# donydchen/matchnerf

Hardware: AMD Instinct MI355X
Metric: rendered rays/sec (3-view, 64 samples/ray) (higher is better)
Workload: dtype f32; 1 GPU

## Files before the change

matchnerf_amd/csrc/api.cpp:

```cpp
#include <string.h>
#include <stdarg.h>
#include <stdio.h>
#include <stdlib.h>

#include <mutex>

#include "common.hpp"
#include "launch_plan.hpp"

static thread_local char g_err[512] = "";

void mnerf_set_error(const char* fmt, ...) {
  va_list ap;
  va_start(ap, fmt);
  vsnprintf(g_err, sizeof(g_err), fmt, ap);
  va_end(ap);
}

extern "C" int mnerf_abi_version(void) { return MNERF_ABI_VERSION; }
extern "C" const char* mnerf_last_error(void) { return g_err; }

extern "C" int64_t mnerf_struct_size(int32_t which) {
  switch (which) {
    case 0: return (int64_t)sizeof(mnerf_view);
    case 1: return (int64_t)sizeof(mnerf_rays);
    case 2: return (int64_t)sizeof(mnerf_scene);
    case 3: return (int64_t)sizeof(mnerf_decoder);
    case 4: return (int64_t)sizeof(mnerf_encoder_layer);
    case 5: return (int64_t)sizeof(mnerf_conv);
    case 6: return (int64_t)sizeof(mnerf_decoder_train);
    case 7: return (int64_t)sizeof(mnerf_encoder_layer_train);
    case 8: return (int64_t)sizeof(mnerf_optim_row);
    case 9: return (int64_t)sizeof(mnerf_optim_group);
    case 10: return (int64_t)sizeof(mnerf_lpips_weights);
    case MNERF_STRUCT_CAMERA: return (int64_t)sizeof(mnerf_camera);
    default: return -1;
  }
}

int mnerf_rays_canonical(const mnerf_rays* rays, mnerf_rays* out, const char* who) {
  MNERF_REQUIRE(rays, MNERF_E_NULL, "%s: rays is NULL", who);
  *out = *rays;
  MNERF_REQUIRE(rays->tgt_height >= 0 && rays->tgt_width >= 0 && (rays->tgt_height == 0) == (rays->tgt_width == 0), MNERF_E_RANGE,
                "%s: target grid %dx%d (both 0 = the views' size, or both >= 1)", who, rays->tgt_height, rays->tgt_width);
  if (rays->tgt_height == 0) out->tgt_height = rays->height, out->tgt_width = rays->width;
  MNERF_REQUIRE(out->tgt_height >= 1 && out->tgt_width >= 1, MNERF_E_RANGE, "%s: target grid %dx%d", who, out->tgt_height,
                out->tgt_width);
  if (!rays->ray_idx && !rays->pose_table && rays->n_rays > 0)
    MNERF_REQUIRE(rays->ray_begin >= 0 && (long long)rays->ray_begin + rays->n_rays <= (long long)out->tgt_height * out->tgt_width,
                  MNERF_E_RANGE, "%s: pixels [%d, %d + %d) outside the %dx%d target grid", who, rays->ray_begin, rays->ray_begin,
                  rays->n_rays, out->tgt_height, out->tgt_width);
  return MNERF_OK;
}

int mnerf_free_rays_canonical(const mnerf_rays* rays, const float* ray_od, mnerf_rays* out, const char* who) {
  MNERF_REQUIRE(rays, MNERF_E_NULL, "%s: rays is NULL", who);
  MNERF_REQUIRE(!rays->ray_idx && !rays->pose_table, MNERF_E_UNSUPPORTED,
                "%s: a ray bundle excludes ray_idx / pose_table (the bundle's rows are the rays)", who);
  MNERF_REQUIRE(rays->n_rays >= 0 && rays->n_samples >= 1, MNERF_E_RANGE, "%s: n_rays=%d S=%d", who, rays->n_rays, rays->n_samples);
  MNERF_REQUIRE(rays->legacy_coord == 0 || rays->n_samples >= 2, MNERF_E_RANGE, "%s: legacy depth sampling needs S >= 2", who);
  if (rays->n_rays > 0) {
    MNERF_REQUIRE(ray_od, MNERF_E_NULL, "%s: ray_od is NULL", who);
    MNERF_REQUIRE(mnerf_aligned16(ray_od), MNERF_E_ALIGN, "%s: ray_od not 16B aligned", who);
  }
  mnerf_rays c = {};
  c.n_rays = rays->n_rays, c.n_samples = rays->n_samples;
  c.legacy_coord = rays->legacy_coord ? 1 : 0, c.depth_inverse = rays->depth_inverse ? 1 : 0;
  c.height = c.tgt_height = rays->height, c.width = c.tgt_width = rays->width;
  c.near_ = rays->near_, c.far_ = rays->far_;
  c.strat_u = rays->strat_u;
  *out = c;
  return MNERF_OK;
}

static int env_int(const char* name, int dflt) {
  const char* e = getenv(name);
  return (e && *e) ? atoi(e) : dflt;
}

static mnerf_tuning read_tuning() {
  mnerf_tuning t;
  t.decoder_grid = env_int("MNERF_DECODER_GRID", 512);
  t.decoder_stagger = env_int("MNERF_DECODER_STAGGER", 16);
  t.decoder_stagger_mode = env_int("MNERF_DECODER_STAGGER_MODE", 0);
  t.cv_variant = env_int("MNERF_CV_VARIANT", 3);
  t.cv_mm = env_int("MNERF_CV_MM", 1);
  t.cv_mm_spw = env_int("MNERF_CV_MM_SPW", 4);
  t.cv_uvpair = env_int("MNERF_CV_UVPAIR", -1);
  t.cv_pair_block = env_int("MNERF_CV_PAIR_BLOCK", -1);
  t.cv_grid = env_int("MNERF_CV_GRID", 0);
  t.wa_min4 = env_int("MNERF_WA_MIN4", 200);
  t.wa_xcd = env_int("MNERF_WA_XCD", 1);
  t.render_fused = env_int("MNERF_RENDER_FUSED", 0);
  t.decoder_pp = env_int("MNERF_DECODER_PP", 1);
  t.decoder_pp_grid = env_int("MNERF_DECODER_PP_GRID", 256);
  t.decoder_pp_max_s = env_int("MNERF_DECODER_PP_MAX_S", 256);
  return t;
}

static mnerf_tuning g_tuning = read_tuning();
static std::mutex g_tuning_lock;
mnerf_tuning mnerf_tune() {
  std::lock_guard<std::mutex> hold(g_tuning_lock);
  return g_tuning;
}

extern "C" int mnerf_debug_set_knob(const char* name, int value, int* old_value) {
  std::lock_guard<std::mutex> hold(g_tuning_lock);
  struct Knob { const char* name; int* slot; };
  const Knob knobs[] = {{"decoder_pp", &g_tuning.decoder_pp}, {"decoder_pp_grid", &g_tuning.decoder_pp_grid},
                        {"decoder_pp_max_s", &g_tuning.decoder_pp_max_s}, {"decoder_grid", &g_tuning.decoder_grid},
                        {"cv_variant", &g_tuning.cv_variant}, {"cv_mm", &g_tuning.cv_mm}, {"cv_mm_spw", &g_tuning.cv_mm_spw}, {"cv_uvpair", &g_tuning.cv_uvpair}, {"cv_pair_block", &g_tuning.cv_pair_block}, {"cv_grid", &g_tuning.cv_grid},
                        {"render_fused", &g_tuning.render_fused}, {"wa_min4", &g_tuning.wa_min4}};
  for (const Knob& k : knobs)
    if (name && strcmp(name, k.name) == 0) {
      if (old_value) *old_value = *k.slot;
      *k.slot = value;
      return MNERF_OK;
    }
  mnerf_set_error("mnerf_debug_set_knob: unknown knob '%s'", name ? name : "(null)");
  return MNERF_E_RANGE;
}

extern "C" int mnerf_debug_launch_plan(const char* what, const int64_t* args, int32_t n_args, int32_t* plan, int32_t n_plan) {
  MNERF_REQUIRE(what && args && plan, MNERF_E_NULL, "mnerf_debug_launch_plan: NULL argument");
  struct Planner { const char* name; int (*fn)(const int64_t*, int32_t, int32_t*, int32_t); };
  const Planner planners[] = {{"conv2d", mnerf_plan_conv2d}, {"conv_gemm", mnerf_plan_conv_gemm}, {"conv_wgrad", mnerf_plan_conv_wgrad},
                              {"instance_norm", mnerf_plan_instance_norm}, {"instance_norm_backward", mnerf_plan_instance_norm},
                              {"window_attention", mnerf_plan_window_attention}};
  for (const Planner& p : planners)
    if (strcmp(what, p.name) == 0) return p.fn(args, n_args, plan, n_plan);
  mnerf_set_error("mnerf_debug_launch_plan: unknown dispatcher '%s'", what);
  return MNERF_E_RANGE;
}

bool mnerf_once_per_device(std::atomic<unsigned long long>& mask) {
  int dev = 0;
  (void)hipGetDevice(&dev);
  const unsigned long long bit = 1ull << (dev & 63);
  return (mask.fetch_or(bit, std::memory_order_relaxed) & bit) == 0;
}
```

matchnerf_amd/csrc/cost_volume_mm.hip:

```cpp
#include <stdlib.h>

#include "cv_walk.hpp"

typedef _Float16 cvm_h8 __attribute__((ext_vector_type(8)));
typedef _Float16 cvm_h2 __attribute__((ext_vector_type(2)));
typedef float cvm_f2 __attribute__((ext_vector_type(2)));
typedef float cvm_f16 __attribute__((ext_vector_type(16)));
typedef unsigned cvm_u4 __attribute__((ext_vector_type(4)));

#define CVM_MAX_MAPS (MNERF_MAX_VIEWS * (MNERF_MAX_VIEWS - 1))
#define CVM_HDR_BYTES 8192
#define CVM_COL_BYTES 1024
#define CVM_TARGET_EXP 15
#define CVM_UV_MAX_VIEWS MNERF_MAX_VIEWS

struct CvmLayout {
  int nrp[2], rs[2];
  size_t map_bytes[2], off[2], total;
};

__host__ __device__ inline CvmLayout cvm_layout(const mnerf_scene& sc) {
  CvmLayout L;
  const size_t maps = (size_t)sc.n_views * (sc.n_views - 1);
  size_t o = CVM_HDR_BYTES;
  for (int s = 0; s < 2; ++s) {
    if (s < sc.n_scales) {
      L.nrp[s] = (sc.fh[s] + 1) / 2 + 1;
      L.rs[s] = sc.fw[s] + 3;
      L.map_bytes[s] = (size_t)L.nrp[s] * L.rs[s] * CVM_COL_BYTES;
    } else {
      L.nrp[s] = L.rs[s] = 0;
      L.map_bytes[s] = 0;
    }
    L.off[s] = o;
    o += L.map_bytes[s] * maps;
  }
  L.total = o;
  return L;
}

__global__ __launch_bounds__(256) void cvm_absmax_kernel(mnerf_scene sc, unsigned* __restrict__ absmax_bits) {
  const int maps = sc.n_views * (sc.n_views - 1);
  const int s = (int)blockIdx.y >= maps ? 1 : 0, m = (int)blockIdx.y - s * maps;
  const size_t n4 = (size_t)sc.fh[s] * sc.fw[s] * (FEAT_C / 4);
  const v4f* src = reinterpret_cast<const v4f*>(sc.feat[s]) + (size_t)m * n4;
  float mx = 0.0f;
  for (size_t i = (size_t)blockIdx.x * 256 + threadIdx.x; i < n4; i += (size_t)gridDim.x * 256) {
    const v4f v = src[i];
    mx = fmaxf(fmaxf(mx, fmaxf(fabsf(v.x), fabsf(v.y))), fmaxf(fabsf(v.z), fabsf(v.w)));
  }
#pragma unroll
  for (int off = 32; off > 0; off >>= 1) mx = fmaxf(mx, __shfl_xor(mx, off, 64));
  if ((threadIdx.x & 63) == 0) atomicMax(absmax_bits + s * CVM_MAX_MAPS + m, __float_as_uint(mx));
}

__device__ __forceinline__ int cvm_gain_exp(float m) {
  if (!(m > 0.0f) || !(m < 3.0e38f)) return 0;
  int e = __builtin_amdgcn_frexp_expf(m);
  e = e < -100 ? -100 : (e > 100 ? 100 : e);
  return CVM_TARGET_EXP - e;
}

__global__ __launch_bounds__(256) void cvm_split_kernel(mnerf_scene sc, char* __restrict__ opnd) {
  const CvmLayout L = cvm_layout(sc);
  const int maps = sc.n_views * (sc.n_views - 1);
  const int s = (int)blockIdx.y >= maps ? 1 : 0, m = (int)blockIdx.y - s * maps;
  const int fh = sc.fh[s], fw = sc.fw[s];
  const int cell = (int)blockIdx.x * 2 + (int)(threadIdx.x >> 7), ch = threadIdx.x & 127;
  if (cell >= L.nrp[s] * L.rs[s]) return;
  const int rp = cell / L.rs[s], x = cell - rp * L.rs[s];
  float* gain = reinterpret_cast<float*>(opnd);
  const unsigned* absmax_bits = reinterpret_cast<const unsigned*>(opnd + 2 * 2 * CVM_MAX_MAPS * 4);
  const int e = cvm_gain_exp(__uint_as_float(absmax_bits[s * CVM_MAX_MAPS + m]));
  const float g = ldexpf(1.0f, e);
  if (cell == 0 && ch == 0) {
    gain[s * CVM_MAX_MAPS + m] = g;
    gain[2 * CVM_MAX_MAPS + s * CVM_MAX_MAPS + m] = ldexpf(1.0f, -e);
  }
  const float* src = sc.feat[s] + (size_t)m * fh * fw * FEAT_C + ch;
  cvm_h2 hi, lo;
#pragma unroll
  for (int r = 0; r < 2; ++r) {
    const int y = 2 * rp + r;
    float v = 0.0f;
    if (y < fh && x < fw) v = src[((size_t)y * fw + x) * FEAT_C];
    v = v * g;
    v = fminf(fmaxf(v, -65504.0f), 65504.0f);
    const _Float16 h = (_Float16)v;
    hi[r] = h;
    lo[r] = (_Float16)(v - (float)h);
  }
  char* dst = opnd + L.off[s] + (size_t)m * L.map_bytes[s] + (size_t)cell * CVM_COL_BYTES + (size_t)ch * 4;
  *reinterpret_cast<cvm_h2*>(dst) = hi;
  *reinterpret_cast<cvm_h2*>(dst + 512) = lo;
}

__device__ __forceinline__ void cvm_swap32(float& a, float& b) {
  asm("s_nop 1\n\tv_permlane32_swap_b32_e32 %0, %1" : "+v"(a), "+v"(b));
}
__device__ __forceinline__ float cvm_fold_pair(float x, float y) {
  cvm_swap32(x, y);
  return x + y;
}

struct CvmTap {
  unsigned xy;
  unsigned c0_hi, c1_hi, c0_lo, c1_lo;
};

__device__ __forceinline__ unsigned cvm_pack_h2(float a, float b) {
  const cvm_f2 ab = {a, b};
  return __builtin_bit_cast(unsigned, __builtin_convertvector(ab, cvm_h2));
}
__device__ __forceinline__ float cvm_resid_lo(float v, unsigned hpk) {
  float r;
  asm("v_fma_mix_f32 %0, %1, 1.0, -%2 op_sel_hi:[0,0,1]" : "=v"(r) : "v"(v), "v"(hpk));
  return r;
}
__device__ __forceinline__ float cvm_resid_hi(float v, unsigned hpk) {
  float r;
  asm("v_fma_mix_f32 %0, %1, 1.0, -%2 op_sel:[0,0,1] op_sel_hi:[0,0,1]" : "=v"(r) : "v"(v), "v"(hpk));
  return r;
// ... 196 lines not shown
    cvm_f16 z;
#pragma unroll
    for (int i = 0; i < 16; ++i) z[i] = 0.0f;
    fa = cvm_mfma(l_a, wah, z);
    fb = cvm_mfma(l_b, wbh, z);
    fa = cvm_mfma(h_a, wal, fa);
    fb = cvm_mfma(h_b, wbl, fb);
    fa = cvm_mfma(h_a, wah, fa);
    fb = cvm_mfma(h_b, wbh, fb);
  };
  auto request = [&](int ct) {
    if constexpr (REQ) {
      cvm_load_ct(ha[ct], la[ct], next_a, ct);
      cvm_load_ct(hb[ct], lb[ct], next_b, ct);
    }
  };
#define CVM_PIN(q) asm volatile("" : "+v"(dot[q]), "+v"(dot[q + 1]), "+v"(na[q]), "+v"(na[q + 1]), "+v"(nb[q]), "+v"(nb[q + 1]));
  if constexpr (MORE) {
    const unsigned loff_a = cvm_lane_off(sa.rs, n, half), loff_b = cvm_lane_off(sb.rs, n, half);
#pragma unroll 1
    for (int ct = 0; ct < 4; ++ct) {
#pragma unroll
      for (int i = 0; i < 16; ++i) fa0[i] = 0.0f, fb0[i] = 0.0f;
      cvm_all_chunks(fa0, sa, tap_a, loff_a, ct, lut, half, fh, fw);
      cvm_all_chunks(fb0, sb, tap_b, loff_b, ct, lut, half, fh, fw);
      float d2[2], a2[2], b2[2];
      cvm_dots(fa0, fb0, d2, a2, b2);
      switch (ct) {
        case 0: dot[0] = d2[0], dot[1] = d2[1], na[0] = a2[0], na[1] = a2[1], nb[0] = b2[0], nb[1] = b2[1]; break;
        case 1: dot[2] = d2[0], dot[3] = d2[1], na[2] = a2[0], na[3] = a2[1], nb[2] = b2[0], nb[3] = b2[1]; break;
        case 2: dot[4] = d2[0], dot[5] = d2[1], na[4] = a2[0], na[5] = a2[1], nb[4] = b2[0], nb[5] = b2[1]; break;
        default: dot[6] = d2[0], dot[7] = d2[1], na[6] = a2[0], na[7] = a2[1], nb[6] = b2[0], nb[7] = b2[1]; break;
      }
    }
#pragma unroll
    for (int ct = 0; ct < 4; ++ct) request(ct);
  } else {
    tile(0, fa0, fb0);
    request(0);
    tile(1, fa1, fb1);
    cvm_dots(fa0, fb0, dot + 0, na + 0, nb + 0);
    CVM_PIN(0)
    request(1);
    tile(2, fa0, fb0);
    cvm_dots(fa1, fb1, dot + 2, na + 2, nb + 2);
    CVM_PIN(2)
    request(2);
    tile(3, fa1, fb1);
    cvm_dots(fa0, fb0, dot + 4, na + 4, nb + 4);
    CVM_PIN(4)
    request(3);
    cvm_dots(fa1, fb1, dot + 6, na + 6, nb + 6);
  }
#undef CVM_PIN
  cvm_cosines(cacc, dot, na, nb, ea2, eb2, G);
}


struct CvmGrid {
  int tile_y0, ntx, n_tiles, nsg, spw;
  int stage_rows;
  int pair_begin, pair_end, a0, b0;
};

__host__ __device__ inline size_t cvm_wave_lds_bytes(int n_views, int n_scales, int cond_stride, int stage_rows) {
  const size_t items = (size_t)n_views * n_scales;
  return (size_t)n_views * 32 * 8 + items * (32 * 16 + 32 * 4 + 16) + (stage_rows ? (size_t)32 * cond_stride * 4 : 0);
}

#define CVM_WAVES_PER_SIMD 2
#define CVM_WG_WAVES 4
#ifdef CVM_STATS
#define CVM_DBG_PARAM , unsigned long long* __restrict__ dbg
#define CVM_T(i)                                                  \
  {                                                               \
    const unsigned long long t_ = __builtin_amdgcn_s_memtime();   \
    st[i] += t_ - t_last;                                         \
    t_last = t_;                                                  \
  }
#else
#define CVM_DBG_PARAM
#define CVM_T(i)
#endif
__global__ __launch_bounds__(64 * CVM_WG_WAVES, CVM_WAVES_PER_SIMD) void cost_volume_mm_kernel(mnerf_scene sc, mnerf_rays R, int cond_stride,
                                                                                 float* __restrict__ cond, const char* __restrict__ opnd,
                                                                                 CvmGrid grid CVM_DBG_PARAM) {
#ifdef CVM_STATS
  unsigned long long st[8] = {0, 0, 0, 0, 0, 0, 0, 0}, t_last = __builtin_amdgcn_s_memtime();
#endif
  extern __shared__ __attribute__((aligned(16))) char cvm_smem[];
  const int lane = threadIdx.x & 63, wave = __builtin_amdgcn_readfirstlane(threadIdx.x >> 6);
  const int n = lane & 31, half = lane >> 5;
  const int S = R.n_samples, V = sc.n_views, NS = sc.n_scales;
  const int W = R.tgt_width, H = R.tgt_height;
  const int Ws = R.width, Hs = R.height;
  const int items = V * NS;
  const CvmLayout L = cvm_layout(sc);
  const float* gain = reinterpret_cast<const float*>(opnd);
  const cvm_u4* lut = reinterpret_cast<const cvm_u4*>(cvm_smem);
  cvm_lut_init(reinterpret_cast<unsigned*>(cvm_smem));
  __syncthreads();
  char* wl = cvm_smem + CVM_LUT_BYTES + (size_t)wave * cvm_wave_lds_bytes(V, NS, cond_stride, grid.stage_rows);
  float2* uv = reinterpret_cast<float2*>(wl);
  cvm_u4* tapw = reinterpret_cast<cvm_u4*>(wl + (size_t)V * 256);
  unsigned* tapxy = reinterpret_cast<unsigned*>(wl + (size_t)V * 256 + (size_t)items * 512);
  int4* boxes = reinterpret_cast<int4*>(wl + (size_t)V * 256 + (size_t)items * 640);
  float* rows = reinterpret_cast<float*>(wl + (size_t)V * 256 + (size_t)items * 656);

  const int nwg = gridDim.x;
  const int xcd = blockIdx.x & 7, lin = blockIdx.x >> 3;
  const int q8 = nwg >> 3, r8 = nwg & 7;
  const int item = (xcd < r8 ? xcd * (q8 + 1) : r8 * (q8 + 1) + (xcd - r8) * q8) + lin;
  const int tile = item / grid.nsg, sg = item - tile * grid.nsg;
  const int tyi = tile / grid.ntx, txi = tile - tyi * grid.ntx;

  const int px = txi * 8 + (n & 7), py = (grid.tile_y0 + tyi) * 4 + (n >> 3);
  const int pix = min(py, H - 1) * W + min(px, W - 1);
  const int ray_geo = pix - R.ray_begin;
  const int ray = max(0, min(ray_geo, R.n_rays - 1));
  const bool row_wr = grid.stage_rows || (px < W && py < H && ray_geo >= 0 && ray_geo < R.n_rays);
  const float wm1 = (float)(Ws - 1), hm1 = (float)(Hs - 1);
  const int G0 = sc.n_group[0], G1 = NS > 1 ? sc.n_group[1] : 0;
  const int sumG = G0 + G1;
  const int n_pairs = V * (V - 1) / 2;
  const float inv_pairs = 1.0f / (float)n_pairs;
  const bool first_block = grid.pair_begin == 0, last_block = grid.pair_end == n_pairs;

  for (int k = 0; k < grid.spw; ++k) {
    const int j = (sg * grid.spw + k) * CVM_WG_WAVES + wave;
    if (j >= S) break;
    float* out = grid.stage_rows ? rows + n * cond_stride : cond + ((size_t)ray * S + j) * cond_stride;
    float wx, wy, wz;
    {
      int rg = ray_geo;
      asm volatile("" : "+v"(rg));
      ray_point(make_ray(R, rg), sample_depth(R, ray, j), wx, wy, wz);
    }

    CVM_T(7)
    cvw_handoff();
    for (int v = half; v < V; v += 2) {
      float u, w_, z;
      project(sc.views[v], wx, wy, wz, wm1, hm1, u, w_, z);
      uv[v * 32 + n] = make_float2(u, w_);
      if (row_wr && first_block) {
        const Bilin b = bilin_setup(u, w_, Hs, Ws);
        const float4* img = reinterpret_cast<const float4*>(sc.images) + (size_t)v * Hs * Ws;
        const float4 t00 = img[b.o00], t01 = img[b.o01], t10 = img[b.o10], t11 = img[b.o11];
        const float gx = u * 2.0f - 1.0f, gy = w_ * 2.0f - 1.0f;
        const float m = (gx > -1.0f && gx < 1.0f && gy > -1.0f && gy < 1.0f) ? 1.0f : 0.0f;
        out[sumG + 3 * v + 0] = bilin4(t00.x, t01.x, t10.x, t11.x, b);
        out[sumG + 3 * v + 1] = bilin4(t00.y, t01.y, t10.y, t11.y, b);
        out[sumG + 3 * v + 2] = bilin4(t00.z, t01.z, t10.z, t11.z, b);
        out[sumG + 3 * V + v] = m;
      }
    }
    if (half == 0 && row_wr && first_block) {
      const int dc = sumG + 4 * V;
      out[dc] = 1.0f;
      for (int c = dc + 1; c < cond_stride; ++c) out[c] = 0.0f;
    }
    cvw_handoff();
    CVM_T(0)

    for (int it = 0; 2 * it < items; ++it) {
      const int i = min(2 * it + half, items - 1);
      const int v = NS == 2 ? i >> 1 : i, s = i - v * NS;
      const float2 p2 = uv[v * 32 + n];
      int x0, y0;
      const int fh_s = s == 0 ? sc.fh[0] : sc.fh[1], fw_s = s == 0 ? sc.fw[0] : sc.fw[1];
      const CvmTap t = cvm_tap(p2.x, p2.y, fh_s, fw_s, x0, y0);
      cvm_u4 wv;
      wv.x = t.c0_hi, wv.y = t.c1_hi, wv.z = t.c0_lo, wv.w = t.c1_lo;
      tapw[i * 32 + n] = wv;
      tapxy[i * 32 + n] = t.xy;
      const int y1 = min(y0 + 1, fh_s - 1), x1 = min(x0 + 1, fw_s - 1);
      int xmin = x0, ymin = y0;
#define CVM_MM_STEP(CTRL)                                                                                                    \
  {                                                                                                                          \
    xmin = min(xmin, __builtin_amdgcn_update_dpp(0x7fffffff, xmin, CTRL, 0xF, 0xF, false));  \
    ymin = min(ymin, __builtin_amdgcn_update_dpp(0x7fffffff, ymin, CTRL, 0xF, 0xF, false));                                         \
  }
      CVM_MM_STEP(0xB1)
      CVM_MM_STEP(0x4E)
      CVM_MM_STEP(0x141)
      CVM_MM_STEP(0x140)
#undef CVM_MM_STEP
      xmin = min(xmin, __builtin_amdgcn_ds_swizzle(xmin, 0x401F));
      ymin = min(ymin, __builtin_amdgcn_ds_swizzle(ymin, 0x401F));
      const int p_lo = ymin >> 1, xb_lo = xmin;
      const int cra = ((y0 >> 1) - p_lo) >> 1, crb = ((y1 >> 1) - p_lo) >> 1;
      const int cxa = (x0 - xb_lo) >> 2, cxb = (x1 - xb_lo) >> 2;
      const unsigned long long ob = __builtin_amdgcn_ballot_w64(crb > 7 || cxb > 7);
      const bool big = (half ? (unsigned)(ob >> 32) : (unsigned)ob) != 0u;
      unsigned long long mk = (1ull << ((8 * cra + cxa) & 63)) | (1ull << ((8 * cra + cxb) & 63)) | (1ull << ((8 * crb + cxa) & 63)) |
                              (1ull << ((8 * crb + cxb) & 63));
      unsigned mlo = (unsigned)mk, mhi = (unsigned)(mk >> 32);
#define CVM_OR_STEP(CTRL)                                                                             \
  {                                                                                                   \
    mlo |= (unsigned)__builtin_amdgcn_update_dpp(0, (int)mlo, CTRL, 0xF, 0xF, false);                 \
    mhi |= (unsigned)__builtin_amdgcn_update_dpp(0, (int)mhi, CTRL, 0xF, 0xF, false);                 \
  }
      CVM_OR_STEP(0xB1)
      CVM_OR_STEP(0x4E)
      CVM_OR_STEP(0x141)
      CVM_OR_STEP(0x140)
#undef CVM_OR_STEP
      mlo |= (unsigned)__builtin_amdgcn_ds_swizzle((int)mlo, 0x401F);
      mhi |= (unsigned)__builtin_amdgcn_ds_swizzle((int)mhi, 0x401F);
      if (n == 0 && 2 * it + half < items) boxes[i] = make_int4(p_lo, xb_lo, big ? 0 : (int)mlo, big ? 0 : (int)mhi);
    }
    cvw_handoff();

    CVM_T(1)
    float c0[4] = {0.f, 0.f, 0.f, 0.f}, c1[4] = {0.f, 0.f, 0.f, 0.f};
    if (!first_block && row_wr) {
#pragma unroll
      for (int i = 0; i < 4; ++i) {
        const int gi = 2 * i + half;
        if (gi < G0) c0[i] = out[gi];
        if (gi < G1) c1[i] = out[G0 + gi];
      }
    }
    auto tap_of = [&](int i) {
      CvmTap t;
      const cvm_u4 wv = tapw[i * 32 + n];
      t.xy = tapxy[i * 32 + n];
      t.c0_hi = wv.x, t.c1_hi = wv.y, t.c0_lo = wv.z, t.c1_lo = wv.w;
      return t;
    };
    auto side_of = [&](const char* map, int view, int s) {
      CvmSide o;
      o.map = map;
      o.rs = s == 0 ? L.rs[0] : L.rs[1];
      o.item = view * NS + s;
      const int4 bx = boxes[o.item];
      o.box.p_lo = __builtin_amdgcn_readfirstlane(bx.x), o.box.xb_lo = __builtin_amdgcn_readfirstlane(bx.y);
      o.box.mask = (unsigned long long)(unsigned)__builtin_amdgcn_readfirstlane(bx.z) |
                   ((unsigned long long)(unsigned)__builtin_amdgcn_readfirstlane(bx.w) << 32);
      o.box.big = o.box.mask == 0;
      o.p = o.box.p_lo, o.xb = o.box.xb_lo;
      if (!o.box.big) {
        unsigned long long m = o.box.mask;
        cvm_pop(m, o.box, o.p, o.xb);
      }
      return o;
    };
    auto first_of = [&](const CvmSide& sd) { return cvm_chunk_base(sd, sd.p, sd.xb) + cvm_lane_off(sd.rs, n, half); };
    auto has_more = [&](const CvmSide& sd) { return sd.box.big || (sd.box.mask & (sd.box.mask - 1)) != 0; };
    const char* mp0 = opnd + L.off[0] + (size_t)(2 * grid.pair_begin) * L.map_bytes[0];
    const char* mp1 = opnd + L.off[1] + (size_t)(2 * grid.pair_begin) * L.map_bytes[1];
    int pr = grid.pair_begin, a = grid.a0, b = grid.b0, s = 0;
    CvmSide sa = side_of(mp0, a, 0), sb = side_of(mp0 + L.map_bytes[0], b, 0);
    cvm_u4 ha[4], la[4], hb[4], lb[4];
    {
      const char* fa_ = first_of(sa);
      const char* fb_ = first_of(sb);
#pragma unroll
      for (int ct = 0; ct < 4; ++ct) cvm_load_ct(ha[ct], la[ct], fa_, ct), cvm_load_ct(hb[ct], lb[ct], fb_, ct);
    }
    const int n_units = (grid.pair_end - grid.pair_begin) * NS;
    auto unit = [&](auto req_tag) {
      constexpr bool REQ = decltype(req_tag)::value;
      CVM_T(2)
      const float ga = gain[s * CVM_MAX_MAPS + 2 * pr], gb = gain[s * CVM_MAX_MAPS + 2 * pr + 1];
      const float ea = 1e-8f * ga, eb = 1e-8f * gb;
      const int G = s == 0 ? G0 : G1;
      const int s_cur = s;
      const int fh_u = s == 0 ? sc.fh[0] : sc.fh[1], fw_u = s == 0 ? sc.fw[0] : sc.fw[1];
      CvmSide na_ = sa, nb_ = sb;
      if constexpr (REQ) {
        if (++s == NS) {
          s = 0, ++pr;
          mp0 += 2 * L.map_bytes[0], mp1 += 2 * L.map_bytes[1];
          if (++b == V) ++a, b = a + 1;
        }
        const char* mpn = s == 0 ? mp0 : mp1;
        na_ = side_of(mpn, a, s);
        nb_ = side_of(mpn + (s == 0 ? L.map_bytes[0] : L.map_bytes[1]), b, s);
      }
      const CvmTap tap_a = tap_of(sa.item), tap_b = tap_of(sb.item);
      float cu[4] = {0.f, 0.f, 0.f, 0.f};
      if (has_more(sa) || has_more(sb))
        cvm_unit_run<true, REQ>(cu, ha, la, hb, lb, sa, sb, tap_a, tap_b, first_of(na_), first_of(nb_), ea * ea, eb * eb, G, lut, n, half, fh_u,
                                fw_u);
      else
        cvm_unit_run<false, REQ>(cu, ha, la, hb, lb, sa, sb, tap_a, tap_b, first_of(na_), first_of(nb_), ea * ea, eb * eb, G, lut, n, half, fh_u,
                                 fw_u);
      if (s_cur == 0) {
#pragma unroll
        for (int i = 0; i < 4; ++i) c0[i] += cu[i];
      } else {
#pragma unroll
        for (int i = 0; i < 4; ++i) c1[i] += cu[i];
      }
      sa = na_, sb = nb_;
      CVM_T(5)
    };
    for (int u = 0; u + 1 < n_units; ++u) unit(std::true_type{});
    if (n_units > 0) unit(std::false_type{});
    if (row_wr) {
#pragma unroll
      for (int i = 0; i < 4; ++i) {
        const int gi = 2 * i + half;
        if (gi < G0) out[gi] = last_block ? c0[i] * inv_pairs : c0[i];
        if (gi < G1) out[G0 + gi] = last_block ? c1[i] * inv_pairs : c1[i];
      }
    }
    cvw_handoff();
    if (grid.stage_rows) {
      const int ppr = cond_stride >> 2;
      const int ppr_sh = (ppr & (ppr - 1)) == 0 ? __builtin_ctz(ppr) : -1;
      for (int c = lane; c < 32 * ppr; c += 64) {
        const int r = ppr_sh >= 0 ? c >> ppr_sh : c / ppr, part = c - r * ppr;
        const int rpx = txi * 8 + (r & 7), rpy = (grid.tile_y0 + tyi) * 4 + (r >> 3);
        const int rpix = rpy * W + rpx;
        if (rpx < W && rpy < H && rpix >= R.ray_begin && rpix < R.ray_begin + R.n_rays)
          *reinterpret_cast<v4f*>(cond + ((size_t)(rpix - R.ray_begin) * S + j) * cond_stride + 4 * part) =
              *reinterpret_cast<const v4f*>(rows + r * cond_stride + 4 * part);
      }
    }
    CVM_T(6)
  }
#ifdef CVM_STATS
  if (dbg && lane == 0) {
    for (int i = 0; i < 8; ++i) atomicAdd(dbg + i, st[i]);
    atomicAdd(dbg + 8, 1ull);
  }
#endif
}

extern "C" int64_t mnerf_cost_volume_operand_bytes(const mnerf_scene* scene) {
  if (!scene || scene->n_views < 2 || scene->n_views > MNERF_MAX_VIEWS || scene->n_scales < 1 || scene->n_scales > 2) return -1;
  return (int64_t)cvm_layout(*scene).total;
}

extern "C" int mnerf_cost_volume_operands(const mnerf_scene* scene, void* opnd, void* stream) {
  MNERF_REQUIRE(scene && opnd, MNERF_E_NULL, "mnerf_cost_volume_operands: NULL argument");
  MNERF_REQUIRE(scene->n_views >= 2 && scene->n_views <= MNERF_MAX_VIEWS, MNERF_E_RANGE, "mnerf_cost_volume_operands: n_views=%d",
                scene->n_views);
  MNERF_REQUIRE(scene->n_scales == 1 || scene->n_scales == 2, MNERF_E_RANGE, "mnerf_cost_volume_operands: n_scales=%d", scene->n_scales);
  MNERF_REQUIRE(mnerf_aligned16(opnd), MNERF_E_ALIGN, "mnerf_cost_volume_operands: buffer not 16B aligned");
  for (int s = 0; s < scene->n_scales; ++s) {
    MNERF_REQUIRE(scene->feat[s], MNERF_E_NULL, "mnerf_cost_volume_operands: feat[%d] is NULL", s);
    MNERF_REQUIRE(mnerf_aligned16(scene->feat[s]), MNERF_E_ALIGN, "mnerf_cost_volume_operands: feat[%d] not 16B aligned", s);
    MNERF_REQUIRE(scene->fh[s] >= 1 && scene->fw[s] >= 1, MNERF_E_RANGE, "mnerf_cost_volume_operands: feature map %d is %dx%d", s,
                  scene->fh[s], scene->fw[s]);
  }
  const CvmLayout L = cvm_layout(*scene);
  const int maps = scene->n_views * (scene->n_views - 1);
  hipStream_t st = (hipStream_t)stream;
  hipError_t e = hipMemsetAsync(opnd, 0, CVM_HDR_BYTES, st);
  if (e != hipSuccess) {
    mnerf_set_error("mnerf_cost_volume_operands: memset failed: %s", hipGetErrorString(e));
    return (int)e;
  }
  unsigned* absmax_bits = reinterpret_cast<unsigned*>(reinterpret_cast<char*>(opnd) + 2 * 2 * CVM_MAX_MAPS * 4);
  hipLaunchKernelGGL(cvm_absmax_kernel, dim3(32, (unsigned)(maps * scene->n_scales)), dim3(256), 0, st, *scene, absmax_bits);
  int cells = 0;
  for (int s = 0; s < scene->n_scales; ++s) cells = cells > L.nrp[s] * L.rs[s] ? cells : L.nrp[s] * L.rs[s];
  hipLaunchKernelGGL(cvm_split_kernel, dim3((unsigned)((cells + 1) / 2), (unsigned)(maps * scene->n_scales)), dim3(256), 0, st, *scene,
                     reinterpret_cast<char*>(opnd));
  return mnerf_check_launch("mnerf_cost_volume_operands");
}

bool mnerf_cost_volume_mm_applies(const mnerf_scene* scene, const mnerf_rays* rays) {
  return scene->feat_op != nullptr && rays->ray_idx == nullptr && rays->pose_table == nullptr;
}

int mnerf_cost_volume_mm_launch(const mnerf_scene* scene, const mnerf_rays* rays, int cond_stride, float* cond, void* stream) {
  MNERF_REQUIRE(mnerf_aligned16(scene->feat_op), MNERF_E_ALIGN, "mnerf_cost_volume: feat_op not 16B aligned");
  const int W = rays->tgt_width;
  const int row_first = rays->ray_begin / W, row_last = (rays->ray_begin + rays->n_rays - 1) / W;
  CvmGrid g;
  g.tile_y0 = row_first / 4;
  g.ntx = (W + 7) / 8;
  g.n_tiles = g.ntx * (row_last / 4 - g.tile_y0 + 1);
  int spw = mnerf_tune().cv_mm_spw;
  if (spw <= 0) spw = 4;
  g.spw = spw;
  g.nsg = (rays->n_samples + CVM_WG_WAVES * spw - 1) / (CVM_WG_WAVES * spw);
  const long long items = (long long)g.n_tiles * g.nsg;
  MNERF_REQUIRE(items < (1ll << 31), MNERF_E_RANGE, "mnerf_cost_volume: %lld work items", items);
  const int n_pairs = scene->n_views * (scene->n_views - 1) / 2;
  int blk = mnerf_tune().cv_pair_block > 0 ? mnerf_tune().cv_pair_block : n_pairs;
  if (scene->n_views <= 5) blk = n_pairs;
  g.stage_rows = blk >= n_pairs &&
                 (2 * (CVM_LUT_BYTES + CVM_WG_WAVES * cvm_wave_lds_bytes(scene->n_views, scene->n_scales, cond_stride, 1)) <= 160 * 1024 ||
                  2 * (CVM_LUT_BYTES + CVM_WG_WAVES * cvm_wave_lds_bytes(scene->n_views, scene->n_scales, cond_stride, 0)) > 160 * 1024);
  const size_t lds = CVM_LUT_BYTES + CVM_WG_WAVES * cvm_wave_lds_bytes(scene->n_views, scene->n_scales, cond_stride, g.stage_rows);
  MNERF_REQUIRE(lds <= 160 * 1024, MNERF_E_UNSUPPORTED, "mnerf_cost_volume: %d views need %zu B of LDS", scene->n_views, lds);
  static std::atomic<unsigned long long> attr_set{0};
  if (mnerf_once_per_device(attr_set))
    (void)hipFuncSetAttribute((const void*)cost_volume_mm_kernel, hipFuncAttributeMaxDynamicSharedMemorySize, 160 * 1024);
#ifdef CVM_STATS
  unsigned long long* dbg = nullptr;
  if (const char* e = getenv("MNERF_CVDBG_PTR")) dbg = (unsigned long long*)strtoull(e, nullptr, 0);
#endif
  int a = 0, b = 1;
  for (int p0 = 0; p0 < n_pairs; p0 += blk) {
    g.pair_begin = p0, g.pair_end = p0 + blk < n_pairs ? p0 + blk : n_pairs, g.a0 = a, g.b0 = b;
#ifdef CVM_STATS
    hipLaunchKernelGGL(cost_volume_mm_kernel, dim3((unsigned)items), dim3(64 * CVM_WG_WAVES), lds, (hipStream_t)stream, *scene, *rays,
                       cond_stride, cond, reinterpret_cast<const char*>(scene->feat_op), g, dbg);
#else
    hipLaunchKernelGGL(cost_volume_mm_kernel, dim3((unsigned)items), dim3(64 * CVM_WG_WAVES), lds, (hipStream_t)stream, *scene, *rays,
                       cond_stride, cond, reinterpret_cast<const char*>(scene->feat_op), g);
#endif
    for (int i = 0; i < blk; ++i)
      if (++b == scene->n_views) ++a, b = a + 1;
  }
  return mnerf_check_launch("mnerf_cost_volume");
}
```

matchnerf_amd/csrc/launch_plan.hpp:

```cpp
#pragma once
#include <stdint.h>

int mnerf_plan_conv2d(const int64_t* args, int32_t n_args, int32_t* plan, int32_t n_plan);
int mnerf_plan_conv_gemm(const int64_t* args, int32_t n_args, int32_t* plan, int32_t n_plan);
int mnerf_plan_conv_wgrad(const int64_t* args, int32_t n_args, int32_t* plan, int32_t n_plan);
int mnerf_plan_instance_norm(const int64_t* args, int32_t n_args, int32_t* plan, int32_t n_plan);
int mnerf_plan_window_attention(const int64_t* args, int32_t n_args, int32_t* plan, int32_t n_plan);
```

Before: 12.85 million rays/s.

## Add compile-time specialized cost-volume kernel for 3 views and 2 scales

Templates the matmul cost-volume kernel on view and scale counts and dispatches a fully static instance for the 3-view, 2-scale case. The pair and scale walk is unrolled at compile time, per-unit gain epsilons are precomputed into scalar registers, box descriptors are hoisted once, and the view projection loop is unrolled. This removes runtime index arithmetic and dynamic pair/scale bookkeeping from the inner loop. The cost is larger code and possibly more register pressure. A launch-plan query and a runtime knob are added to turn the path on or off.

```diff
diff --git a/matchnerf_amd/csrc/api.cpp b/matchnerf_amd/csrc/api.cpp
--- a/matchnerf_amd/csrc/api.cpp
+++ b/matchnerf_amd/csrc/api.cpp
@@ -104,13 +104,18 @@
   std::lock_guard<std::mutex> hold(g_tuning_lock);
   return g_tuning;
 }
+static int g_cv_mm_static = env_int("MNERF_CV_MM_STATIC", 1);
+int mnerf_cv_mm_static() {
+  std::lock_guard<std::mutex> hold(g_tuning_lock);
+  return g_cv_mm_static;
+}
 
 extern "C" int mnerf_debug_set_knob(const char* name, int value, int* old_value) {
   std::lock_guard<std::mutex> hold(g_tuning_lock);
   struct Knob { const char* name; int* slot; };
   const Knob knobs[] = {{"decoder_pp", &g_tuning.decoder_pp}, {"decoder_pp_grid", &g_tuning.decoder_pp_grid},
                         {"decoder_pp_max_s", &g_tuning.decoder_pp_max_s}, {"decoder_grid", &g_tuning.decoder_grid},
-                        {"cv_variant", &g_tuning.cv_variant}, {"cv_mm", &g_tuning.cv_mm}, {"cv_mm_spw", &g_tuning.cv_mm_spw}, {"cv_uvpair", &g_tuning.cv_uvpair}, {"cv_pair_block", &g_tuning.cv_pair_block}, {"cv_grid", &g_tuning.cv_grid},
+                        {"cv_variant", &g_tuning.cv_variant}, {"cv_mm", &g_tuning.cv_mm}, {"cv_mm_spw", &g_tuning.cv_mm_spw}, {"cv_mm_static", &g_cv_mm_static}, {"cv_uvpair", &g_tuning.cv_uvpair}, {"cv_pair_block", &g_tuning.cv_pair_block}, {"cv_grid", &g_tuning.cv_grid},
                         {"render_fused", &g_tuning.render_fused}, {"wa_min4", &g_tuning.wa_min4}};
   for (const Knob& k : knobs)
     if (name && strcmp(name, k.name) == 0) {
@@ -127,7 +132,7 @@
   struct Planner { const char* name; int (*fn)(const int64_t*, int32_t, int32_t*, int32_t); };
   const Planner planners[] = {{"conv2d", mnerf_plan_conv2d}, {"conv_gemm", mnerf_plan_conv_gemm}, {"conv_wgrad", mnerf_plan_conv_wgrad},
                               {"instance_norm", mnerf_plan_instance_norm}, {"instance_norm_backward", mnerf_plan_instance_norm},
-                              {"window_attention", mnerf_plan_window_attention}};
+                              {"window_attention", mnerf_plan_window_attention}, {"cost_volume_mm", mnerf_plan_cost_volume_mm}};
   for (const Planner& p : planners)
     if (strcmp(what, p.name) == 0) return p.fn(args, n_args, plan, n_plan);
   mnerf_set_error("mnerf_debug_launch_plan: unknown dispatcher '%s'", what);
diff --git a/matchnerf_amd/csrc/cost_volume_mm.hip b/matchnerf_amd/csrc/cost_volume_mm.hip
--- a/matchnerf_amd/csrc/cost_volume_mm.hip
+++ b/matchnerf_amd/csrc/cost_volume_mm.hip
@@ -1,6 +1,10 @@
 #include <stdlib.h>
 
+#include <type_traits>
+#include <utility>
+
 #include "cv_walk.hpp"
+#include "launch_plan.hpp"
 
 typedef _Float16 cvm_h8 __attribute__((ext_vector_type(8)));
 typedef _Float16 cvm_h2 __attribute__((ext_vector_type(2)));
@@ -19,12 +23,12 @@
   size_t map_bytes[2], off[2], total;
 };
 
-__host__ __device__ inline CvmLayout cvm_layout(const mnerf_scene& sc) {
+__host__ __device__ inline CvmLayout cvm_layout_of(const mnerf_scene& sc, int n_views, int n_scales) {
   CvmLayout L;
-  const size_t maps = (size_t)sc.n_views * (sc.n_views - 1);
+  const size_t maps = (size_t)n_views * (n_views - 1);
   size_t o = CVM_HDR_BYTES;
   for (int s = 0; s < 2; ++s) {
-    if (s < sc.n_scales) {
+    if (s < n_scales) {
       L.nrp[s] = (sc.fh[s] + 1) / 2 + 1;
       L.rs[s] = sc.fw[s] + 3;
       L.map_bytes[s] = (size_t)L.nrp[s] * L.rs[s] * CVM_COL_BYTES;
@@ -38,6 +42,7 @@
   L.total = o;
   return L;
 }
+__host__ __device__ inline CvmLayout cvm_layout(const mnerf_scene& sc) { return cvm_layout_of(sc, sc.n_views, sc.n_scales); }
 
 __global__ __launch_bounds__(256) void cvm_absmax_kernel(mnerf_scene sc, unsigned* __restrict__ absmax_bits) {
   const int maps = sc.n_views * (sc.n_views - 1);
@@ -400,20 +405,37 @@
 #define CVM_DBG_PARAM
 #define CVM_T(i)
 #endif
+struct CvmUnitDesc {
+  int a, b, s, pr;
+};
+template <int V_, int NS_>
+constexpr CvmUnitDesc cvm_unit_desc(int u) {
+  CvmUnitDesc d = {0, 1, u % NS_, u / NS_};
+  for (int i = 0; i < d.pr; ++i)
+    if (++d.b == V_) ++d.a, d.b = d.a + 1;
+  return d;
+}
+template <class F, int... I>
+__device__ __forceinline__ void cvm_each_index(F&& f, std::integer_sequence<int, I...>) {
+  (f(std::integral_constant<int, I>{}), ...);
+}
+
+template <int V_, int NS_>
 __global__ __launch_bounds__(64 * CVM_WG_WAVES, CVM_WAVES_PER_SIMD) void cost_volume_mm_kernel(mnerf_scene sc, mnerf_rays R, int cond_stride,
                                                                                  float* __restrict__ cond, const char* __restrict__ opnd,
                                                                                  CvmGrid grid CVM_DBG_PARAM) {
 #ifdef CVM_STATS
   unsigned long long st[8] = {0, 0, 0, 0, 0, 0, 0, 0}, t_last = __builtin_amdgcn_s_memtime();
 #endif
+  constexpr bool ST = V_ != 0;
   extern __shared__ __attribute__((aligned(16))) char cvm_smem[];
   const int lane = threadIdx.x & 63, wave = __builtin_amdgcn_readfirstlane(threadIdx.x >> 6);
   const int n = lane & 31, half = lane >> 5;
-  const int S = R.n_samples, V = sc.n_views, NS = sc.n_scales;
+  const int S = R.n_samples, V = ST ? V_ : sc.n_views, NS = ST ? NS_ : sc.n_scales;
   const int W = R.tgt_width, H = R.tgt_height;
   const int Ws = R.width, Hs = R.height;
   const int items = V * NS;
-  const CvmLayout L = cvm_layout(sc);
+  const CvmLayout L = cvm_layout_of(sc, V, NS);
   const float* gain = reinterpret_cast<const float*>(opnd);
   const cvm_u4* lut = reinterpret_cast<const cvm_u4*>(cvm_smem);
   cvm_lut_init(reinterpret_cast<unsigned*>(cvm_smem));
@@ -441,12 +463,30 @@
   const int G0 = sc.n_group[0], G1 = NS > 1 ? sc.n_group[1] : 0;
   const int sumG = G0 + G1;
   const int n_pairs = V * (V - 1) / 2;
-  const float inv_pairs = 1.0f / (float)n_pairs;
-  const bool first_block = grid.pair_begin == 0, last_block = grid.pair_end == n_pairs;
-
+  const float inv_pairs = 1.0f / (float)(sc.n_views * (sc.n_views - 1) / 2);
+  const bool first_block = ST || grid.pair_begin == 0, last_block = ST || grid.pair_end == n_pairs;
+  constexpr int NU = ST ? V_ * (V_ - 1) / 2 * NS_ : 1;
+  float ea2_st[NU], eb2_st[NU];
+  if constexpr (ST) {
+#pragma unroll
+    for (int u = 0; u < NU; ++u) {
+      const int slot = (u % NS_) * CVM_MAX_MAPS + 2 * (u / NS_);
+      const float ea = 1e-8f * gain[slot], eb = 1e-8f * gain[slot + 1];
+      ea2_st[u] = __builtin_bit_cast(float, __builtin_amdgcn_readfirstlane(__builtin_bit_cast(int, ea * ea)));
+      eb2_st[u] = __builtin_bit_cast(float, __builtin_amdgcn_readfirstlane(__builtin_bit_cast(int, eb * eb)));
+    }
+  }
+
+  const int n_w = n, half_w = half;
   for (int k = 0; k < grid.spw; ++k) {
     const int j = (sg * grid.spw + k) * CVM_WG_WAVES + wave;
     if (j >= S) break;
+    int n = n_w, half = half_w;
+    if constexpr (ST) {
+      int lane_k = lane;
+      asm volatile("" : "+v"(lane_k));
+      n = lane_k & 31, half = lane_k >> 5;
+    }
     float* out = grid.stage_rows ? rows + n * cond_stride : cond + ((size_t)ray * S + j) * cond_stride;
     float wx, wy, wz;
     {
@@ -457,7 +497,7 @@
 
     CVM_T(7)
     cvw_handoff();
-    for (int v = half; v < V; v += 2) {
+    auto pass1_view = [&](int v) {
       float u, w_, z;
       project(sc.views[v], wx, wy, wz, wm1, hm1, u, w_, z);
       uv[v * 32 + n] = make_float2(u, w_);
@@ -472,6 +512,17 @@
         out[sumG + 3 * v + 2] = bilin4(t00.z, t01.z, t10.z, t11.z, b);
         out[sumG + 3 * V + v] = m;
       }
+    };
+    if constexpr (ST) {
+#pragma unroll
+      for (int v0 = 0; v0 < V_; v0 += 2) {
+        if (v0 + 1 < V_)
+          pass1_view(v0 + half);
+        else if (half == 0)
+          pass1_view(v0);
+      }
+    } else {
+      for (int v = half; v < V; v += 2) pass1_view(v);
     }
     if (half == 0 && row_wr && first_block) {
       const int dc = sumG + 4 * V;
@@ -481,9 +532,7 @@
     cvw_handoff();
     CVM_T(0)
 
-    for (int it = 0; 2 * it < items; ++it) {
-      const int i = min(2 * it + half, items - 1);
-      const int v = NS == 2 ? i >> 1 : i, s = i - v * NS;
+    auto pass1b_item = [&](int i, int v, int s, bool store) {
       const float2 p2 = uv[v * 32 + n];
       int x0, y0;
       const int fh_s = s == 0 ? sc.fh[0] : sc.fh[1], fw_s = s == 0 ? sc.fw[0] : sc.fw[1];
@@ -526,7 +575,17 @@
 #undef CVM_OR_STEP
       mlo |= (unsigned)__builtin_amdgcn_ds_swizzle((int)mlo, 0x401F);
       mhi |= (unsigned)__builtin_amdgcn_ds_swizzle((int)mhi, 0x401F);
-      if (n == 0 && 2 * it + half < items) boxes[i] = make_int4(p_lo, xb_lo, big ? 0 : (int)mlo, big ? 0 : (int)mhi);
+      if (n == 0 && store) boxes[i] = make_int4(p_lo, xb_lo, big ? 0 : (int)mlo, big ? 0 : (int)mhi);
+    };
+    if constexpr (ST && NS_ == 2) {
+#pragma unroll
+      for (int it = 0; it < V_; ++it) pass1b_item(2 * it + half, it, half, true);
+    } else {
+      for (int it = 0; 2 * it < items; ++it) {
+        const int i = min(2 * it + half, items - 1);
+        const int v = NS == 2 ? i >> 1 : i, s = i - v * NS;
+        pass1b_item(i, v, s, 2 * it + half < items);
+      }
     }
     cvw_handoff();
 
@@ -547,15 +606,13 @@
       t.c0_hi = wv.x, t.c1_hi = wv.y, t.c0_lo = wv.z, t.c1_lo = wv.w;
       return t;
     };
-    auto side_of = [&](const char* map, int view, int s) {
+    auto side_of_box = [&](const char* map, int rs, int item, const int4& bx) {
       CvmSide o;
       o.map = map;
-      o.rs = s == 0 ? L.rs[0] : L.rs[1];
-      o.item = view * NS + s;
-      const int4 bx = boxes[o.item];
-      o.box.p_lo = __builtin_amdgcn_readfirstlane(bx.x), o.box.xb_lo = __builtin_amdgcn_readfirstlane(bx.y);
-      o.box.mask = (unsigned long long)(unsigned)__builtin_amdgcn_readfirstlane(bx.z) |
-                   ((unsigned long long)(unsigned)__builtin_amdgcn_readfirstlane(bx.w) << 32);
+      o.rs = rs;
+      o.item = item;
+      o.box.p_lo = bx.x, o.box.xb_lo = bx.y;
+      o.box.mask = (unsigned long long)(unsigned)bx.z | ((unsigned long long)(unsigned)bx.w << 32);
       o.box.big = o.box.mask == 0;
       o.p = o.box.p_lo, o.xb = o.box.xb_lo;
       if (!o.box.big) {
@@ -564,59 +621,137 @@
       }
       return o;
     };
+    auto side_of = [&](const char* map, int view, int s) {
+      const int4 bx = boxes[view * NS + s];
+      return side_of_box(map, s == 0 ? L.rs[0] : L.rs[1], view * NS + s,
+                         make_int4(__builtin_amdgcn_readfirstlane(bx.x), __builtin_amdgcn_readfirstlane(bx.y),
+                                   __builtin_amdgcn_readfirstlane(bx.z), __builtin_amdgcn_readfirstlane(bx.w)));
+    };
     auto first_of = [&](const CvmSide& sd) { return cvm_chunk_base(sd, sd.p, sd.xb) + cvm_lane_off(sd.rs, n, half); };
     auto has_more = [&](const CvmSide& sd) { return sd.box.big || (sd.box.mask & (sd.box.mask - 1)) != 0; };
-    const char* mp0 = opnd + L.off[0] + (size_t)(2 * grid.pair_begin) * L.map_bytes[0];
-    const char* mp1 = opnd + L.off[1] + (size_t)(2 * grid.pair_begin) * L.map_bytes[1];
-    int pr = grid.pair_begin, a = grid.a0, b = grid.b0, s = 0;
-    CvmSide sa = side_of(mp0, a, 0), sb = side_of(mp0 + L.map_bytes[0], b, 0);
     cvm_u4 ha[4], la[4], hb[4], lb[4];
-    {
-      const char* fa_ = first_of(sa);
-      const char* fb_ = first_of(sb);
-#pragma unroll
-      for (int ct = 0; ct < 4; ++ct) cvm_load_ct(ha[ct], la[ct], fa_, ct), cvm_load_ct(hb[ct], lb[ct], fb_, ct);
-    }
-    const int n_units = (grid.pair_end - grid.pair_begin) * NS;
-    auto unit = [&](auto req_tag) {
-      constexpr bool REQ = decltype(req_tag)::value;
-      CVM_T(2)
-      const float ga = gain[s * CVM_MAX_MAPS + 2 * pr], gb = gain[s * CVM_MAX_MAPS + 2 * pr + 1];
-      const float ea = 1e-8f * ga, eb = 1e-8f * gb;
-      const int G = s == 0 ? G0 : G1;
-      const int s_cur = s;
-      const int fh_u = s == 0 ? sc.fh[0] : sc.fh[1], fw_u = s == 0 ? sc.fw[0] : sc.fw[1];
-      CvmSide na_ = sa, nb_ = sb;
-      if constexpr (REQ) {
-        if (++s == NS) {
-          s = 0, ++pr;
-          mp0 += 2 * L.map_bytes[0], mp1 += 2 * L.map_bytes[1];
-          if (++b == V) ++a, b = a + 1;
+    if constexpr (ST) {
+      static_assert(NS_ == 2, "the static instance selects between a pair's two scales");
+      constexpr int NI = V_ * NS_, NP = NU / NS_;
+      int4 bxs[NI];
+#pragma unroll
+      for (int i = 0; i < NI; ++i) {
+        const int4 bx = boxes[i];
+        bxs[i].x = __builtin_amdgcn_readfirstlane(bx.x), bxs[i].y = __builtin_amdgcn_readfirstlane(bx.y);
+        bxs[i].z = __builtin_amdgcn_readfirstlane(bx.z), bxs[i].w = __builtin_amdgcn_readfirstlane(bx.w);
+      }
+      auto side_st = [&](bool first, auto ux, auto uy, auto side_tag) {
+        constexpr CvmUnitDesc X = cvm_unit_desc<V_, NS_>(decltype(ux)::value), Y = cvm_unit_desc<V_, NS_>(decltype(uy)::value);
+        constexpr int SIDE = decltype(side_tag)::value;
+        constexpr int IX = (SIDE ? X.b : X.a) * NS_ + X.s, IY = (SIDE ? Y.b : Y.a) * NS_ + Y.s;
+        const int4 bx = make_int4(first ? bxs[IX].x : bxs[IY].x, first ? bxs[IX].y : bxs[IY].y, first ? bxs[IX].z : bxs[IY].z,
+                                  first ? bxs[IX].w : bxs[IY].w);
+        const size_t mb = first ? L.map_bytes[X.s] : L.map_bytes[Y.s];
+        const char* map = opnd + (first ? L.off[X.s] : L.off[Y.s]) + (size_t)(first ? 2 * X.pr + SIDE : 2 * Y.pr + SIDE) * mb;
+        return side_of_box(map, first ? L.rs[X.s] : L.rs[Y.s], first ? IX : IY, bx);
+      };
+      using cvm_side_a = std::integral_constant<int, 0>;
+      using cvm_side_b = std::integral_constant<int, 1>;
+      {
+        using U0 = std::integral_constant<int, 0>;
+        const char* fa_ = first_of(side_st(true, U0{}, U0{}, cvm_side_a{}));
+        const char* fb_ = first_of(side_st(true, U0{}, U0{}, cvm_side_b{}));
+#pragma unroll
+        for (int ct = 0; ct < 4; ++ct) cvm_load_ct(ha[ct], la[ct], fa_, ct), cvm_load_ct(hb[ct], lb[ct], fb_, ct);
+      }
+      auto unit_st = [&](auto pr_tag, auto req_tag, int s) {
+        constexpr int PR = decltype(pr_tag)::value;
+        constexpr bool REQ = decltype(req_tag)::value;
+        using U0 = std::integral_constant<int, 2 * PR>;
+        using U1 = std::integral_constant<int, 2 * PR + 1>;
+        using U2 = std::integral_constant<int, (2 * PR + 2 < NU ? 2 * PR + 2 : NU - 1)>;
+        CVM_T(2)
+        const bool s0 = s == 0;
+        const CvmSide sa = side_st(s0, U0{}, U1{}, cvm_side_a{}), sb = side_st(s0, U0{}, U1{}, cvm_side_b{});
+        const char *next_a = nullptr, *next_b = nullptr;
+        if constexpr (REQ) {
+          next_a = first_of(side_st(s0, U1{}, U2{}, cvm_side_a{}));
+          next_b = first_of(side_st(s0, U1{}, U2{}, cvm_side_b{}));
         }
-        const char* mpn = s == 0 ? mp0 : mp1;
-        na_ = side_of(mpn, a, s);
-        nb_ = side_of(mpn + (s == 0 ? L.map_bytes[0] : L.map_bytes[1]), b, s);
-      }
-      const CvmTap tap_a = tap_of(sa.item), tap_b = tap_of(sb.item);
-      float cu[4] = {0.f, 0.f, 0.f, 0.f};
-      if (has_more(sa) || has_more(sb))
-        cvm_unit_run<true, REQ>(cu, ha, la, hb, lb, sa, sb, tap_a, tap_b, first_of(na_), first_of(nb_), ea * ea, eb * eb, G, lut, n, half, fh_u,
-                                fw_u);
-      else
-        cvm_unit_run<false, REQ>(cu, ha, la, hb, lb, sa, sb, tap_a, tap_b, first_of(na_), first_of(nb_), ea * ea, eb * eb, G, lut, n, half, fh_u,
-                                 fw_u);
-      if (s_cur == 0) {
-#pragma unroll
-        for (int i = 0; i < 4; ++i) c0[i] += cu[i];
-      } else {
-#pragma unroll
-        for (int i = 0; i < 4; ++i) c1[i] += cu[i];
-      }
-      sa = na_, sb = nb_;
-      CVM_T(5)
-    };
-    for (int u = 0; u + 1 < n_units; ++u) unit(std::true_type{});
-    if (n_units > 0) unit(std::false_type{});
+        const CvmTap tap_a = tap_of(sa.item), tap_b = tap_of(sb.item);
+        const int G = s0 ? G0 : G1;
+        const float ea2 = s0 ? ea2_st[2 * PR] : ea2_st[2 * PR + 1], eb2 = s0 ? eb2_st[2 * PR] : eb2_st[2 * PR + 1];
+        float cu[4] = {0.f, 0.f, 0.f, 0.f};
+        if (has_more(sa) || has_more(sb)) {
+          const int fh_u = s0 ? sc.fh[0] : sc.fh[1], fw_u = s0 ? sc.fw[0] : sc.fw[1];
+          cvm_unit_run<true, REQ>(cu, ha, la, hb, lb, sa, sb, tap_a, tap_b, next_a, next_b, ea2, eb2, G, lut, n, half, fh_u, fw_u);
+        } else {
+          cvm_unit_run<false, REQ>(cu, ha, la, hb, lb, sa, sb, tap_a, tap_b, next_a, next_b, ea2, eb2, G, lut, n, half, 0, 0);
+        }
+        if (s0) {
+#pragma unroll
+          for (int i = 0; i < 4; ++i) c0[i] += cu[i];
+        } else {
+#pragma unroll
+          for (int i = 0; i < 4; ++i) c1[i] += cu[i];
+        }
+        CVM_T(5)
+      };
+      cvm_each_index(
+          [&](auto pr_tag) {
+            constexpr bool LAST = decltype(pr_tag)::value == NP - 1;
+#pragma unroll 1
+            for (int s = 0; s < (LAST ? NS_ - 1 : NS_); ++s) unit_st(pr_tag, std::true_type{}, s);
+            if constexpr (LAST) unit_st(pr_tag, std::false_type{}, NS_ - 1);
+          },
+          std::make_integer_sequence<int, NP>{});
+    } else {
+      const char* mp0 = opnd + L.off[0] + (size_t)(2 * grid.pair_begin) * L.map_bytes[0];
+      const char* mp1 = opnd + L.off[1] + (size_t)(2 * grid.pair_begin) * L.map_bytes[1];
+      int pr = grid.pair_begin, a = grid.a0, b = grid.b0, s = 0;
+      CvmSide sa = side_of(mp0, a, 0), sb = side_of(mp0 + L.map_bytes[0], b, 0);
+      {
+        const char* fa_ = first_of(sa);
+        const char* fb_ = first_of(sb);
+#pragma unroll
+        for (int ct = 0; ct < 4; ++ct) cvm_load_ct(ha[ct], la[ct], fa_, ct), cvm_load_ct(hb[ct], lb[ct], fb_, ct);
+      }
+      const int n_units = (grid.pair_end - grid.pair_begin) * NS;
+      auto unit = [&](auto req_tag) {
+        constexpr bool REQ = decltype(req_tag)::value;
+        CVM_T(2)
+        const float ga = gain[s * CVM_MAX_MAPS + 2 * pr], gb = gain[s * CVM_MAX_MAPS + 2 * pr + 1];
+        const float ea = 1e-8f * ga, eb = 1e-8f * gb;
+        const int G = s == 0 ? G0 : G1;
+        const int s_cur = s;
+        const int fh_u = s == 0 ? sc.fh[0] : sc.fh[1], fw_u = s == 0 ? sc.fw[0] : sc.fw[1];
+        CvmSide na_ = sa, nb_ = sb;
+        if constexpr (REQ) {
+          if (++s == NS) {
+            s = 0, ++pr;
+            mp0 += 2 * L.map_bytes[0], mp1 += 2 * L.map_bytes[1];
+            if (++b == V) ++a, b = a + 1;
+          }
+          const char* mpn = s == 0 ? mp0 : mp1;
+          na_ = side_of(mpn, a, s);
+          nb_ = side_of(mpn + (s == 0 ? L.map_bytes[0] : L.map_bytes[1]), b, s);
+        }
+        const CvmTap tap_a = tap_of(sa.item), tap_b = tap_of(sb.item);
+        float cu[4] = {0.f, 0.f, 0.f, 0.f};
+        if (has_more(sa) || has_more(sb))
+          cvm_unit_run<true, REQ>(cu, ha, la, hb, lb, sa, sb, tap_a, tap_b, first_of(na_), first_of(nb_), ea * ea, eb * eb, G, lut, n, half, fh_u,
+                                  fw_u);
+        else
+          cvm_unit_run<false, REQ>(cu, ha, la, hb, lb, sa, sb, tap_a, tap_b, first_of(na_), first_of(nb_), ea * ea, eb * eb, G, lut, n, half, fh_u,
+                                   fw_u);
+        if (s_cur == 0) {
+#pragma unroll
+          for (int i = 0; i < 4; ++i) c0[i] += cu[i];
+        } else {
+#pragma unroll
+          for (int i = 0; i < 4; ++i) c1[i] += cu[i];
+        }
+        sa = na_, sb = nb_;
+        CVM_T(5)
+      };
+      for (int u = 0; u + 1 < n_units; ++u) unit(std::true_type{});
+      if (n_units > 0) unit(std::false_type{});
+    }
     if (row_wr) {
 #pragma unroll
       for (int i = 0; i < 4; ++i) {
@@ -684,6 +819,26 @@
 
 bool mnerf_cost_volume_mm_applies(const mnerf_scene* scene, const mnerf_rays* rays) {
   return scene->feat_op != nullptr && rays->ray_idx == nullptr && rays->pose_table == nullptr;
+}
+
+static int cvm_pair_block(int n_views) {
+  const int n_pairs = n_views * (n_views - 1) / 2;
+  int blk = mnerf_tune().cv_pair_block > 0 ? mnerf_tune().cv_pair_block : n_pairs;
+  if (n_views <= 5) blk = n_pairs;
+  return blk;
+}
+static bool cvm_takes_static(int n_views, int n_scales, int blk) {
+  return n_views == 3 && n_scales == 2 && blk >= n_views * (n_views - 1) / 2 && mnerf_cv_mm_static() != 0;
+}
+
+int mnerf_plan_cost_volume_mm(const int64_t* a, int32_t n_args, int32_t* plan, int32_t n_plan) {
+  const char* who = "mnerf_debug_launch_plan(cost_volume_mm)";
+  MNERF_REQUIRE(n_args == 2 && n_plan >= 2, MNERF_E_RANGE, "%s: takes 2 arguments and fills 2 values, got %d and %d", who, n_args, n_plan);
+  MNERF_REQUIRE(a[0] >= 2 && a[0] <= MNERF_MAX_VIEWS && (a[1] == 1 || a[1] == 2), MNERF_E_RANGE, "%s: n_views=%lld n_scales=%lld", who,
+                (long long)a[0], (long long)a[1]);
+  const int blk = cvm_pair_block((int)a[0]);
+  plan[0] = cvm_takes_static((int)a[0], (int)a[1], blk) ? 1 : 0, plan[1] = blk;
+  return MNERF_OK;
 }
 
 int mnerf_cost_volume_mm_launch(const mnerf_scene* scene, const mnerf_rays* rays, int cond_stride, float* cond, void* stream) {
@@ -701,16 +856,17 @@
   const long long items = (long long)g.n_tiles * g.nsg;
   MNERF_REQUIRE(items < (1ll << 31), MNERF_E_RANGE, "mnerf_cost_volume: %lld work items", items);
   const int n_pairs = scene->n_views * (scene->n_views - 1) / 2;
-  int blk = mnerf_tune().cv_pair_block > 0 ? mnerf_tune().cv_pair_block : n_pairs;
-  if (scene->n_views <= 5) blk = n_pairs;
+  const int blk = cvm_pair_block(scene->n_views);
   g.stage_rows = blk >= n_pairs &&
                  (2 * (CVM_LUT_BYTES + CVM_WG_WAVES * cvm_wave_lds_bytes(scene->n_views, scene->n_scales, cond_stride, 1)) <= 160 * 1024 ||
                   2 * (CVM_LUT_BYTES + CVM_WG_WAVES * cvm_wave_lds_bytes(scene->n_views, scene->n_scales, cond_stride, 0)) > 160 * 1024);
   const size_t lds = CVM_LUT_BYTES + CVM_WG_WAVES * cvm_wave_lds_bytes(scene->n_views, scene->n_scales, cond_stride, g.stage_rows);
   MNERF_REQUIRE(lds <= 160 * 1024, MNERF_E_UNSUPPORTED, "mnerf_cost_volume: %d views need %zu B of LDS", scene->n_views, lds);
-  static std::atomic<unsigned long long> attr_set{0};
-  if (mnerf_once_per_device(attr_set))
-    (void)hipFuncSetAttribute((const void*)cost_volume_mm_kernel, hipFuncAttributeMaxDynamicSharedMemorySize, 160 * 1024);
+  const bool st = cvm_takes_static(scene->n_views, scene->n_scales, blk);
+  auto* kernel = st ? cost_volume_mm_kernel<3, 2> : cost_volume_mm_kernel<0, 0>;
+  static std::atomic<unsigned long long> attr_set{0}, attr_set_static{0};
+  if (mnerf_once_per_device(st ? attr_set_static : attr_set))
+    (void)hipFuncSetAttribute((const void*)kernel, hipFuncAttributeMaxDynamicSharedMemorySize, 160 * 1024);
 #ifdef CVM_STATS
   unsigned long long* dbg = nullptr;
   if (const char* e = getenv("MNERF_CVDBG_PTR")) dbg = (unsigned long long*)strtoull(e, nullptr, 0);
@@ -719,11 +875,11 @@
   for (int p0 = 0; p0 < n_pairs; p0 += blk) {
     g.pair_begin = p0, g.pair_end = p0 + blk < n_pairs ? p0 + blk : n_pairs, g.a0 = a, g.b0 = b;
 #ifdef CVM_STATS
-    hipLaunchKernelGGL(cost_volume_mm_kernel, dim3((unsigned)items), dim3(64 * CVM_WG_WAVES), lds, (hipStream_t)stream, *scene, *rays,
-                       cond_stride, cond, reinterpret_cast<const char*>(scene->feat_op), g, dbg);
+    hipLaunchKernelGGL(kernel, dim3((unsigned)items), dim3(64 * CVM_WG_WAVES), lds, (hipStream_t)stream, *scene, *rays, cond_stride, cond,
+                       reinterpret_cast<const char*>(scene->feat_op), g, dbg);
 #else
-    hipLaunchKernelGGL(cost_volume_mm_kernel, dim3((unsigned)items), dim3(64 * CVM_WG_WAVES), lds, (hipStream_t)stream, *scene, *rays,
-                       cond_stride, cond, reinterpret_cast<const char*>(scene->feat_op), g);
+    hipLaunchKernelGGL(kernel, dim3((unsigned)items), dim3(64 * CVM_WG_WAVES), lds, (hipStream_t)stream, *scene, *rays, cond_stride, cond,
+                       reinterpret_cast<const char*>(scene->feat_op), g);
 #endif
     for (int i = 0; i < blk; ++i)
       if (++b == scene->n_views) ++a, b = a + 1;
diff --git a/matchnerf_amd/csrc/launch_plan.hpp b/matchnerf_amd/csrc/launch_plan.hpp
--- a/matchnerf_amd/csrc/launch_plan.hpp
+++ b/matchnerf_amd/csrc/launch_plan.hpp
@@ -6,3 +6,5 @@
 int mnerf_plan_conv_wgrad(const int64_t* args, int32_t n_args, int32_t* plan, int32_t n_plan);
 int mnerf_plan_instance_norm(const int64_t* args, int32_t n_args, int32_t* plan, int32_t n_plan);
 int mnerf_plan_window_attention(const int64_t* args, int32_t n_args, int32_t* plan, int32_t n_plan);
+int mnerf_plan_cost_volume_mm(const int64_t* args, int32_t n_args, int32_t* plan, int32_t n_plan);
+int mnerf_cv_mm_static();
```

Measured after the change: 12.81 million rays/s. Within noise of the previous version (-0.3%).
